# sreeramkannan/Shannon

Hardware: AMD Instinct MI355X
Metric: reads/sec k-mer->graph->path-decompose, 2x100bp k=25 (higher is better)
Workload: dtype u64

## Files before the change

### shannon_amd/csrc/common.h

```cpp
#pragma once
#include <hip/hip_runtime.h>
#include <stdint.h>
#include <stdlib.h>
#include <string>
#include <vector>
#include <mutex>
#include "../../include/shannon_hip.h"

hipError_t shn_counted_memcpy(const char* file, int line, void* dst, const void* src, size_t n, hipMemcpyKind kind, hipStream_t s);
hipError_t shn_counted_memset(const char* file, int line, void* dst, int value, size_t n, hipStream_t s);
#define hipMemcpyAsync(...) shn_counted_memcpy(__FILE__, __LINE__, __VA_ARGS__)
#define hipMemsetAsync(...) shn_counted_memset(__FILE__, __LINE__, __VA_ARGS__)

#define SHN_WAVE 64

static inline const char* shn_env_str(const char* name) { return getenv(name); }
static inline bool shn_env_set(const char* name) { return shn_env_str(name) != nullptr; }
static inline bool shn_env_flag(const char* name, bool dflt) {
  const char* v = shn_env_str(name);
  return !v ? dflt : dflt ? v[0] != '0' : v[0] == '1';
}
static inline uint64_t shn_env_u64(const char* name, uint64_t dflt, uint64_t lo = 0, uint64_t hi = ~0ULL) {
  const char* v = shn_env_str(name);
  if (!v) return dflt;
// ... 323 lines not shown
                   int bit_lo, int bit_hi);

int shn_sort_keys(shn_ctx* ctx, uint64_t* keys, uint64_t* keys_tmp, uint64_t n, int bit_lo, int bit_hi, uint64_t** sorted);

static inline uint64_t cdiv(uint64_t a, uint64_t b) { return (a + b - 1) / b; }

struct ShnDevBufs {
  std::vector<void*> p;
  hipStream_t stream;
  explicit ShnDevBufs(hipStream_t s) : stream(s) {}
  template <class T> hipError_t get(T** out, size_t bytes) { hipError_t e = shn_dev_malloc_on((void**)out, bytes, stream); if (e == hipSuccess) p.push_back((void*)*out); return e; }
  ~ShnDevBufs() { for (void* q : p) shn_dev_free_on(q, stream); }
};
void shn_contig_ids(hipStream_t s, const uint64_t* d_off, uint64_t n_contigs, uint32_t* d_cid);
int shn_sorted_windows(shn_ctx* ctx, ShnDevBufs& bufs, const uint8_t* d_bases, const uint64_t* d_off, const uint32_t* d_cid, const int32_t* d_use,
                       uint64_t total, int k, uint64_t** keys, uint32_t** vals, uint64_t* n_out);
```

### shannon_amd/csrc/contig_gpu.hip

```cpp
#include "contig_graph.h"
#include <atomic>
#include <mutex>

namespace {

#define CG_BLK 256

__global__ void cg_cid_kernel(const uint64_t* __restrict__ off, uint64_t n_cand, uint32_t* __restrict__ cid) {
  const uint64_t c = ((uint64_t)blockIdx.x * blockDim.x + threadIdx.x) >> 6;
  if (c >= n_cand) return;
  const uint64_t lo = off[c], hi = off[c + 1];
  for (uint64_t g = lo + (threadIdx.x & 63); g < hi; g += 64) cid[g] = (uint32_t)c;
}

__global__ void cg_flag_kernel(const uint8_t* __restrict__ bases, const uint64_t* __restrict__ off, const uint32_t* __restrict__ cid,
                               const int32_t* __restrict__ use, uint64_t total, int k, uint32_t* __restrict__ flag) {
  for (uint64_t g = (uint64_t)blockIdx.x * blockDim.x + threadIdx.x; g < total; g += (uint64_t)gridDim.x * blockDim.x) {
    const uint32_t c = cid[g];
    flag[g] = (g + (uint64_t)k <= off[c + 1] && (!use || use[c] != 0)) ? 1u : 0u;
  }
}

__device__ __forceinline__ uint32_t cg_code(uint8_t b) { return b == 'A' ? 0u : b == 'C' ? 1u : b == 'G' ? 2u : b == 'T' ? 3u : 4u; }

__global__ void cg_keys_kernel(const uint8_t* __restrict__ bases, const uint32_t* __restrict__ flag, const uint64_t* __restrict__ pos,
                               uint64_t total, int k, uint64_t* __restrict__ keys, uint32_t* __restrict__ vals,
                               unsigned long long* __restrict__ n_bad) {
  for (uint64_t g = (uint64_t)blockIdx.x * blockDim.x + threadIdx.x; g < total; g += (uint64_t)gridDim.x * blockDim.x) {
    if (!flag[g]) continue;
    uint64_t key = 0;
    bool bad = false;
    for (int j = 0; j < k; j++) { const uint32_t c = cg_code(bases[g + j]); bad |= c > 3; key = (key << 2) | (uint64_t)(c & 3); }
// ... 246 lines not shown
    const uint32_t f = (e - i > 1 && cid[(uint32_t)w] != cid[(uint32_t)last]) ? 1u : 0u;
    for (uint64_t j = i; j < e; j++) flag[j] = f;
  }
}
__global__ void cg_compact_packed_kernel(const uint64_t* __restrict__ words, const uint32_t* __restrict__ flag, const uint64_t* __restrict__ pos, uint64_t n,
                                         uint64_t* __restrict__ okeys, uint32_t* __restrict__ ovals) {
  for (uint64_t i = (uint64_t)blockIdx.x * blockDim.x + threadIdx.x; i < n; i += (uint64_t)gridDim.x * blockDim.x)
    if (flag[i]) { const uint64_t w = words[i]; okeys[pos[i]] = w >> 32; ovals[pos[i]] = (uint32_t)w; }
}
__global__ void cg_compact_kernel(const uint64_t* __restrict__ keys, const uint32_t* __restrict__ vals, const uint32_t* __restrict__ flag,
                                  const uint64_t* __restrict__ pos, uint64_t n, uint64_t* __restrict__ okeys, uint32_t* __restrict__ ovals) {
  for (uint64_t i = (uint64_t)blockIdx.x * blockDim.x + threadIdx.x; i < n; i += (uint64_t)gridDim.x * blockDim.x)
    if (flag[i]) { okeys[pos[i]] = keys[i]; ovals[pos[i]] = vals[i]; }
}

static inline uint32_t grid_for(uint64_t n) { return (uint32_t)std::min<uint64_t>(std::max<uint64_t>(cdiv(n, CG_BLK), 1), 1u << 20); }

}

void shn_contig_ids(hipStream_t s, const uint64_t* d_off, uint64_t n_contigs, uint32_t* d_cid) {
  if (n_contigs) hipLaunchKernelGGL(cg_cid_kernel, dim3((uint32_t)cdiv(n_contigs * 64, CG_BLK)), dim3(CG_BLK), 0, s, d_off, n_contigs, d_cid);
}

int shn_sorted_windows(shn_ctx* ctx, ShnDevBufs& bufs, const uint8_t* d_bases, const uint64_t* d_off, const uint32_t* d_cid,
                          const int32_t* d_use, uint64_t total, int k, uint64_t** keys, uint32_t** vals, uint64_t* n_out) {
  hipStream_t s = ctx->stream; shn_use_stream(s);
  uint32_t* d_flag; uint64_t* d_pos; unsigned long long* d_bad;
  HIP_TRY(bufs.get(&d_flag, (total + 1) * 4));
  HIP_TRY(bufs.get(&d_pos, (total + 2) * 8));
  HIP_TRY(bufs.get(&d_bad, 8));
  HIP_TRY(hipMemsetAsync(d_bad, 0, 8, s));
  hipLaunchKernelGGL(cg_flag_kernel, dim3(grid_for(total)), dim3(CG_BLK), 0, s, d_bases, d_off, d_cid, d_use, total, k, d_flag);
  uint64_t nv = 0;
  int rc = shn_device_scan_u32(ctx, d_flag, total, d_pos, &nv);
  if (rc) return rc;
  *n_out = nv;
  *keys = nullptr; *vals = nullptr;
  if (!nv) return SHN_OK;
  uint64_t *k1, *k2; uint32_t *v1, *v2;
  HIP_TRY(bufs.get(&k1, nv * 8)); HIP_TRY(bufs.get(&k2, nv * 8)); HIP_TRY(bufs.get(&v1, nv * 4)); HIP_TRY(bufs.get(&v2, nv * 4));
  hipLaunchKernelGGL(cg_keys_kernel, dim3(grid_for(total)), dim3(CG_BLK), 0, s, d_bases, d_flag, d_pos, total, k, k1, v1, d_bad);
  unsigned long long bad = 0;
  HIP_TRY(hipMemcpyAsync(&bad, d_bad, 8, hipMemcpyDeviceToHost, s));
  HIP_TRY(hipStreamSynchronize(s));
  if (bad) return shn_fail(SHN_ERR_ARG, "shn_contig_stage: contig with a base outside ACGT");
  if ((rc = shn_sort_pairs(ctx, k1, v1, k2, v2, nv, 0, 2 * k))) return rc;
  *keys = k1; *vals = v1;
  return SHN_OK;
}

static int sorted_windows_packed(shn_ctx* ctx, ShnDevBufs& bufs, const uint8_t* d_bases, const uint64_t* d_off, const uint32_t* d_cid, uint64_t total, int k,
                                 uint64_t** words, uint64_t* n_out) {
  hipStream_t s = ctx->stream; shn_use_stream(s);
  uint32_t* d_flag; uint64_t* d_pos; unsigned long long* d_bad;
  HIP_TRY(bufs.get(&d_flag, (total + 1) * 4));
  HIP_TRY(bufs.get(&d_pos, (total + 2) * 8));
  HIP_TRY(bufs.get(&d_bad, 8));
  HIP_TRY(hipMemsetAsync(d_bad, 0, 8, s));
  hipLaunchKernelGGL(cg_flag_kernel, dim3(grid_for(total)), dim3(CG_BLK), 0, s, d_bases, d_off, d_cid, (const int32_t*)nullptr, total, k, d_flag);
  uint64_t nv = 0;
  int rc = shn_device_scan_u32(ctx, d_flag, total, d_pos, &nv);
  if (rc) return rc;
  *n_out = nv;
  *words = nullptr;
  if (!nv) return SHN_OK;
  uint64_t *w1, *w2;
  HIP_TRY(bufs.get(&w1, nv * 8)); HIP_TRY(bufs.get(&w2, nv * 8));
  hipLaunchKernelGGL(cg_keys_packed_kernel, dim3(grid_for(total)), dim3(CG_BLK), 0, s, d_bases, d_flag, d_pos, total, k, w1, d_bad);
  unsigned long long bad = 0;
  HIP_TRY(hipMemcpyAsync(&bad, d_bad, 8, hipMemcpyDeviceToHost, s));
  HIP_TRY(hipStreamSynchronize(s));
  if (bad) return shn_fail(SHN_ERR_ARG, "shn_contig_stage: contig with a base outside ACGT");
  return shn_sort_keys(ctx, w1, w2, nv, 32, 32 + 2 * k, words);
}
// ... 34 lines not shown
  uint32_t max_len = 0;
  for (uint64_t c = 0; c < n_cand; c++) max_len = std::max<uint32_t>(max_len, (uint32_t)(off[c + 1] - off[c]));
  if (n_cand >= (1u << 21) || max_len >= (1u << 21)) {
    std::vector<uint8_t> fetched;
    if (!bases) {
      fetched.resize(total);
      HIP_TRY(hipMemcpyAsync(fetched.data(), d_bases, total, hipMemcpyDeviceToHost, s));
      HIP_TRY(hipStreamSynchronize(s));
      bases = fetched.data();
    }
    G->add(bases, off, n_cand, accepted_out, best_counts_out);
    *out = G; guard.g = nullptr;
    return SHN_OK;
  }
  uint64_t n_rounds = 0, n_blocks = 0, n_list_rounds = 0;
  {
    ShnDevBufs tmp(s);
    uint64_t* keys = nullptr; uint32_t* vals = nullptr; uint64_t* words = nullptr; uint64_t nv = 0;
    int rc;
    const bool shared_only = shn_env_flag("SHN_CONTIG_SHARED", true);
    const bool packed = r <= 16 && shared_only && shn_env_flag("SHN_CONTIG_PACKED", true);
    { TimerRegion ts(ctx, T_CG_SORT);
      rc = packed ? sorted_windows_packed(ctx, tmp, d_bases, d_off, d_cid, total, r, &words, &nv)
                  : shn_sorted_windows(ctx, tmp, d_bases, d_off, d_cid, nullptr, total, r, &keys, &vals, &nv);
      ts.bytes(packed ? nv * (1 + 8 + (uint64_t)((2 * r + 7) / 8) * 16) : nv * (1 + 12 + (uint64_t)((2 * r + 7) / 8) * 24)); }
    if (rc) return rc;
    lap("r-mer sort (GPU)");
    if (nv > 1 && shared_only) {
      uint32_t* d_f0; uint64_t* d_p0; uint64_t ns0 = 0;
      ShnDevBufs scratch(s);
      HIP_TRY(scratch.get(&d_f0, (nv + 1) * 4));
      HIP_TRY(scratch.get(&d_p0, (nv + 2) * 8));
      if (packed) hipLaunchKernelGGL(cg_shared_packed_kernel, dim3(grid_for(nv)), dim3(CG_BLK), 0, s, words, nv, d_cid, d_f0);
      else hipLaunchKernelGGL(cg_shared_kernel, dim3(grid_for(nv)), dim3(CG_BLK), 0, s, keys, vals, nv, d_cid, d_f0);
      if ((rc = shn_device_scan_u32(ctx, d_f0, nv, d_p0, &ns0))) return rc;
      uint64_t* ok = nullptr; uint32_t* ov = nullptr;
      HIP_TRY(tmp.get(&ok, (ns0 + 1) * 8)); HIP_TRY(tmp.get(&ov, (ns0 + 1) * 4));
      if (ns0 && packed) hipLaunchKernelGGL(cg_compact_packed_kernel, dim3(grid_for(nv)), dim3(CG_BLK), 0, s, words, d_f0, d_p0, nv, ok, ov);
      else if (ns0) hipLaunchKernelGGL(cg_compact_kernel, dim3(grid_for(nv)), dim3(CG_BLK), 0, s, keys, vals, d_f0, d_p0, nv, ok, ov);
      if (dbg) fprintf(stderr, "[contig_stage]   %llu of %llu r-mer windows lie in runs that span two candidates\n", (unsigned long long)ns0, (unsigned long long)nv);
      keys = ok; vals = ov; nv = ns0;
      lap("shared r-mer runs (GPU)");
    } else if (packed && nv == 1) {
      nv = 0;
    }
    uint8_t *d_acc, *d_hit; uint32_t *d_scid, *d_flag, *d_acand, *d_cov, *d_ovf; uint64_t *d_apos, *d_akey; int32_t* d_bestc;
    unsigned long long *d_best, *d_chg;
    HIP_TRY(tmp.get(&d_acc, n_cand + 1)); HIP_TRY(tmp.get(&d_hit, total + 64)); HIP_TRY(tmp.get(&d_scid, (nv + 1) * 4));
    HIP_TRY(tmp.get(&d_flag, (nv + 1) * 4)); HIP_TRY(tmp.get(&d_acand, (nv + 1) * 4)); HIP_TRY(tmp.get(&d_cov, (n_cand + 1) * 4));
    HIP_TRY(tmp.get(&d_ovf, 64)); HIP_TRY(tmp.get(&d_apos, (nv + 2) * 8)); HIP_TRY(tmp.get(&d_akey, (nv + 1) * 8));
    HIP_TRY(tmp.get(&d_bestc, (n_cand + 1) * 4)); HIP_TRY(tmp.get(&d_best, (n_cand + 1) * 8)); HIP_TRY(tmp.get(&d_chg, 64));
    uint8_t *d_aff, *d_chgf; uint32_t* d_aval;
    HIP_TRY(tmp.get(&d_aval, (nv + 1) * 4));
    HIP_TRY(tmp.get(&d_aff, n_cand + 1)); HIP_TRY(tmp.get(&d_chgf, n_cand + 1));
    HIP_TRY(hipMemsetAsync(d_chgf, 0, n_cand + 1, s));
    const bool incremental = shn_env_u64("SHN_CONTIG_INCREMENTAL", 1) != 0;
    HIP_TRY(hipMemsetAsync(d_acc, 0, n_cand + 1, s));
    HIP_TRY(hipMemsetAsync(d_bestc, 0, (n_cand + 1) * 4, s));
    if (nv) hipLaunchKernelGGL(cg_scid_kernel, dim3(grid_for(nv)), dim3(CG_BLK), 0, s, vals, d_cid, nv, d_scid);
    const uint64_t list_max = shn_env_u64("SHN_CONTIG_LIST_MAX", 20000);
    uint32_t *d_pos_of = nullptr, *d_clist = nullptr, *d_alist = nullptr, *d_nlist = nullptr;
    if (list_max && nv && nv < 0xFFFFFFF0ULL) {
      HIP_TRY(tmp.get(&d_pos_of, (total + 1) * 4)); HIP_TRY(tmp.get(&d_clist, (n_cand + 1) * 4)); HIP_TRY(tmp.get(&d_alist, (n_cand + 1) * 4)); HIP_TRY(tmp.get(&d_nlist, 64));
      HIP_TRY(hipMemsetAsync(d_pos_of, 0xFF, (total + 1) * 4, s));
      hipLaunchKernelGGL(cg_pos_of_kernel, dim3(grid_for(nv)), dim3(CG_BLK), 0, s, vals, nv, d_pos_of);
    }
    int lg_slots = 22;
    while (lg_slots < 28 && (1ULL << lg_slots) < nv / 4) lg_slots++;
// ... 88 lines not shown
        if (dbg) fprintf(stderr, "[contig_stage]   block [%llu,%llu) round %d: %llu accepted entries, %llu decisions changed\n", (unsigned long long)lo,
                         (unsigned long long)hi, round, (unsigned long long)na, changed);
        if (!changed) break;
        if (round >= max_rounds && hi - lo > 1) {
          HIP_TRY(hipMemsetAsync(d_aff + lo + (hi - lo) / 2, 0, hi - (lo + (hi - lo) / 2), s));
          hi = lo + (hi - lo) / 2;
          HIP_TRY(hipMemsetAsync(d_acc + hi, 0, n_cand - hi, s));
          HIP_TRY(hipMemsetAsync(d_aff + lo, 1, hi - lo, s));
          round = 0;
        }
      }
      n_blocks++;
      lo = hi;
      bsize = std::min<uint64_t>(bsize * 2, std::max<uint64_t>(blk0, n_cand / 4));
    }
    HIP_TRY(hipMemcpyAsync(acc.data(), d_acc, n_cand, hipMemcpyDeviceToHost, s));
    HIP_TRY(hipMemcpyAsync(best_counts_out, d_bestc, n_cand * 4, hipMemcpyDeviceToHost, s));
    HIP_TRY(hipStreamSynchronize(s));
  }
  std::vector<int32_t> use(n_cand);
  int32_t n_acc = 0;
  for (uint64_t c = 0; c < n_cand; c++) { use[c] = acc[c] ? ++n_acc : 0; accepted_out[c] = use[c]; }
  if (dbg) fprintf(stderr, "[contig_stage] %llu candidates (%llu bases): %llu blocks, %llu rounds (%llu of them candidate by candidate), accepted %d\n",
                   (unsigned long long)n_cand, (unsigned long long)total, (unsigned long long)n_blocks, (unsigned long long)n_rounds, (unsigned long long)n_list_rounds, n_acc);
  lap("duplicate_check rounds (GPU)");

  G->idx = n_acc;
  G->conns.assign((size_t)n_acc + 1, Conn());
  G->n_cand_total = n_cand;
  const int C = k1 - 1;
  if (n_acc > 1) {
    int32_t* d_use;
    HIP_TRY(bufs.get(&d_use, n_cand * 4));
    HIP_TRY(hipMemcpyAsync(d_use, use.data(), n_cand * 4, hipMemcpyHostToDevice, s));
    ShnDevBufs tmp(s);
    uint64_t* keys; uint32_t* vals; uint64_t nv = 0;
    int rc = shn_sorted_windows(ctx, tmp, d_bases, d_off, d_cid, d_use, total, C, &keys, &vals, &nv);
    if (rc) return rc;
    uint64_t ns = 0;
    std::vector<uint64_t> hk; std::vector<uint32_t> hg;
    if (nv > 1) {
      uint32_t* d_flag; uint64_t* d_pos;
      HIP_TRY(tmp.get(&d_flag, (nv + 1) * 4));
      HIP_TRY(tmp.get(&d_pos, (nv + 2) * 8));
      hipLaunchKernelGGL(cg_shared_kernel, dim3(grid_for(nv)), dim3(CG_BLK), 0, s, keys, vals, nv, d_cid, d_flag);
      if ((rc = shn_device_scan_u32(ctx, d_flag, nv, d_pos, &ns))) return rc;
      if (ns) {
        uint64_t* ok; uint32_t* ov;
        HIP_TRY(tmp.get(&ok, ns * 8)); HIP_TRY(tmp.get(&ov, ns * 4));
        hipLaunchKernelGGL(cg_compact_kernel, dim3(grid_for(nv)), dim3(CG_BLK), 0, s, keys, vals, d_flag, d_pos, nv, ok, ov);
        hk.resize(ns); hg.resize(ns);
        HIP_TRY(hipMemcpyAsync(hk.data(), ok, ns * 8, hipMemcpyDeviceToHost, s));
        HIP_TRY(hipMemcpyAsync(hg.data(), ov, ns * 4, hipMemcpyDeviceToHost, s));
        HIP_TRY(hipStreamSynchronize(s));
      }
    }
    if (dbg) fprintf(stderr, "[contig_stage]   %llu of %llu K-mer windows of the accepted contigs lie in runs that span two of them\n", (unsigned long long)ns, (unsigned long long)nv);
    lap("K-mer sort + shared runs (GPU)");
    if (ns) {
      std::vector<uint32_t> run(ns), ea(ns), ep(ns), run_start;
      for (uint64_t e = 0; e < ns; e++) {
        if (e == 0 || hk[e] != hk[e - 1]) run_start.push_back((uint32_t)e);
        run[e] = (uint32_t)run_start.size() - 1;
      }
      run_start.push_back((uint32_t)ns);
      std::vector<uint32_t> order(ns), order2(ns);
      {
        for (uint64_t e = 0; e < ns; e++) order[e] = (uint32_t)e;
        std::vector<uint32_t> cnt(2049);
        for (int pass = 0; pass < 3; pass++) {
          const int sh = 11 * pass;
          if (sh && (total >> sh) == 0) break;
// ... 97 lines not shown
```

### shannon_amd/csrc/probe_gpu.hip

```cpp
#include "common.h"
#include "runs.h"
#include <algorithm>
#include <cstring>
#include <map>

#define PG_BLK 256

struct shn_probe {
  shn_table* table = nullptr;
  std::vector<uint32_t> set_off, set_mem;
};

namespace {

__global__ void pg_head_kernel(const uint64_t* __restrict__ keys, const uint32_t* __restrict__ vals, const uint32_t* __restrict__ cid,
                               const uint32_t* __restrict__ part_of, uint64_t n, uint32_t* __restrict__ head, uint32_t* __restrict__ multi) {
  SHN_GRID_FOR(i, n) {
    if (i && keys[i] == keys[i - 1]) { head[i] = 0; multi[i] = 0; continue; }
    head[i] = 1;
    uint64_t e = i + 1;
    while (e < n && keys[e] == keys[i]) e++;
    multi[i] = part_of[cid[vals[i]]] != part_of[cid[vals[e - 1]]] ? 1u : 0u;
  }
}
// ... 38 lines not shown
                                const uint32_t* __restrict__ part_of, const uint32_t* __restrict__ multi, const uint64_t* __restrict__ hpos,
                                uint64_t n, unsigned long long* __restrict__ n_out, uint64_t cap, uint32_t* __restrict__ o_uidx, uint32_t* __restrict__ o_part) {
  SHN_GRID_FOR(i, n) {
    if (!multi[i]) continue;
    uint32_t p1 = 0, p2 = 0;
    if (pg_run_parts(keys, vals, cid, part_of, n, i, p1, p2) < 3) continue;
    for (uint64_t e = i; e < n && keys[e] == keys[i]; e++) {
      const unsigned long long at = atomicAdd(n_out, 1ULL);
      if (at < cap) { o_uidx[at] = (uint32_t)hpos[i]; o_part[at] = part_of[cid[vals[e]]]; }
    }
  }
}
__global__ void pg_patch_kernel(const uint32_t* __restrict__ uidx, const uint32_t* __restrict__ setid, uint64_t n, uint32_t* __restrict__ uvals) {
  SHN_GRID_FOR(i, n) uvals[uidx[i]] = setid[i] + 1;
}
}

extern "C" void shn_probe_destroy(shn_probe* p) { if (p) { shn_table_destroy(p->table); delete p; } }
extern "C" const shn_table* shn_probe_table(const shn_probe* p) { return p ? p->table : nullptr; }
extern "C" uint32_t shn_probe_n_sets(const shn_probe* p) { return p ? (uint32_t)(p->set_off.size() - 1) : 0; }
extern "C" uint64_t shn_probe_n_members(const shn_probe* p) { return p ? p->set_mem.size() : 0; }
extern "C" int shn_probe_sets(const shn_probe* p, uint32_t* set_off, uint32_t* set_mem) {
  if (!p || !set_off || !set_mem) return shn_fail(SHN_ERR_ARG, "shn_probe_sets: NULL argument");
  std::copy(p->set_off.begin(), p->set_off.end(), set_off);
  std::copy(p->set_mem.begin(), p->set_mem.end(), set_mem);
  return SHN_OK;
}

extern "C" int shn_probe_build(shn_ctx* ctx, const uint8_t* bases, const uint64_t* off, uint64_t n_contigs, const uint32_t* part_of, uint32_t n_parts,
                               int k1, shn_probe** out) {
  if (!ctx || !out || (n_contigs && (!bases || !off || !part_of)) || k1 < 2 || k1 > 32) return shn_fail(SHN_ERR_ARG, "shn_probe_build: bad argument");
  *out = nullptr;
  const uint64_t total = n_contigs ? off[n_contigs] : 0;
  if (total >= 0xFFFFFFF0ULL) return shn_fail(SHN_ERR_OVERFLOW, "shn_probe_build: more than 2^32 contig bases");
  for (uint64_t c = 0; c < n_contigs; c++)
    if (part_of[c] >= n_parts || (c && part_of[c] < part_of[c - 1])) return shn_fail(SHN_ERR_ARG, "shn_probe_build: part_of must be ascending and < n_parts");
  SHN_ENTER(ctx);
  shn_stage_begin(ctx);
  hipStream_t s = ctx->stream;
  shn_probe* P = new shn_probe();
  struct Guard { shn_probe* p; ~Guard() { shn_probe_destroy(p); } } guard{P};
  P->set_off.resize(n_parts + 1);
  P->set_mem.resize(n_parts);
  for (uint32_t p = 0; p <= n_parts; p++) P->set_off[p] = p;
  for (uint32_t p = 0; p < n_parts; p++) P->set_mem[p] = p;
  ShnDevBufs B(ctx->stream);
  uint64_t* ukeys = nullptr; uint32_t* uvals = nullptr;
  uint64_t nu = 0;
  if (total) {
    uint8_t* d_bases; uint64_t* d_off; uint32_t *d_cid, *d_part;
    HIP_TRY(B.get(&d_bases, total + 64)); HIP_TRY(B.get(&d_off, (n_contigs + 1) * 8)); HIP_TRY(B.get(&d_cid, (total + 1) * 4)); HIP_TRY(B.get(&d_part, n_contigs * 4));
    HIP_TRY(hipMemcpyAsync(d_bases, bases, total, hipMemcpyHostToDevice, s));
    HIP_TRY(hipMemcpyAsync(d_off, off, (n_contigs + 1) * 8, hipMemcpyHostToDevice, s));
    HIP_TRY(hipMemcpyAsync(d_part, part_of, n_contigs * 4, hipMemcpyHostToDevice, s));
    shn_contig_ids(s, d_off, n_contigs, d_cid);
    uint64_t* keys; uint32_t* vals; uint64_t nv = 0;
    int rc = shn_sorted_windows(ctx, B, d_bases, d_off, d_cid, nullptr, total, k1, &keys, &vals, &nv);
    if (rc) return rc;
    if (nv) {
      uint32_t *d_head, *d_multi; uint64_t *d_hpos;
      HIP_TRY(B.get(&d_head, (nv + 1) * 4)); HIP_TRY(B.get(&d_multi, (nv + 1) * 4)); HIP_TRY(B.get(&d_hpos, (nv + 2) * 8));
      hipLaunchKernelGGL(pg_head_kernel, dim3(shn_grid(nv, PG_BLK)), dim3(PG_BLK), 0, s, keys, vals, d_cid, d_part, nv, d_head, d_multi);
      if ((rc = shn_device_scan_u32(ctx, d_head, nv, d_hpos, &nu))) return rc;
      HIP_TRY(B.get(&ukeys, (nu + 1) * 8)); HIP_TRY(B.get(&uvals, (nu + 1) * 4));
      hipLaunchKernelGGL(pg_unique_kernel, dim3(shn_grid(nv, PG_BLK)), dim3(PG_BLK), 0, s, keys, vals, d_cid, d_part, d_head, d_hpos, nv, ukeys, uvals);
      unsigned long long* d_nm; uint32_t *d_mu = nullptr, *d_mp = nullptr;
      HIP_TRY(B.get(&d_nm, 8));
      {
        uint64_t *d_pair, *d_pair2, *d_dist; uint32_t *d_pu, *d_pu2;
        HIP_TRY(B.get(&d_pair, (nu + 1) * 8)); HIP_TRY(B.get(&d_pair2, (nu + 1) * 8)); HIP_TRY(B.get(&d_pu, (nu + 1) * 4)); HIP_TRY(B.get(&d_pu2, (nu + 1) * 4));
        HIP_TRY(hipMemsetAsync(d_nm, 0, 8, s));
        hipLaunchKernelGGL(pg_pair_kernel, dim3(shn_grid(nv, PG_BLK)), dim3(PG_BLK), 0, s, keys, vals, d_cid, d_part, d_multi, d_hpos, nv, d_nm, d_pair, d_pu);
        unsigned long long n_pair = 0;
        HIP_TRY(hipMemcpyAsync(&n_pair, d_nm, 8, hipMemcpyDeviceToHost, s));
        HIP_TRY(hipStreamSynchronize(s));
        if (n_pair) {
          if ((rc = shn_sort_pairs(ctx, d_pair, d_pu, d_pair2, d_pu2, n_pair, 0, 32 + shn_bits_for(n_parts)))) return rc;
          ShnRuns runs;
          if ((rc = shn_sorted_runs(ctx, B, d_pair, n_pair, 0, 0, &runs))) return rc;
          const uint64_t n_dist = runs.n_runs;
          HIP_TRY(B.get(&d_dist, (n_dist + 1) * 8));
          const uint32_t first_sid = (uint32_t)(P->set_off.size() - 1);
          hipLaunchKernelGGL(pg_pair_patch_kernel, dim3(shn_grid(n_pair, PG_BLK)), dim3(PG_BLK), 0, s, d_pair, d_pu, runs.head, runs.pos, (uint64_t)n_pair, first_sid, uvals, d_dist);
          std::vector<uint64_t> dist(n_dist);
          HIP_TRY(hipMemcpyAsync(dist.data(), d_dist, n_dist * 8, hipMemcpyDeviceToHost, s));
          HIP_TRY(hipStreamSynchronize(s));
          for (uint64_t pr : dist) {
            P->set_mem.push_back((uint32_t)(pr >> 32)); P->set_mem.push_back((uint32_t)pr);
            P->set_off.push_back((uint32_t)P->set_mem.size());
          }
        }
      }
      uint64_t cap = 1 << 16;
      unsigned long long nm = 0;
      while (true) {
        HIP_TRY(B.get(&d_mu, cap * 4)); HIP_TRY(B.get(&d_mp, cap * 4));
        HIP_TRY(hipMemsetAsync(d_nm, 0, 8, s));
        hipLaunchKernelGGL(pg_multi_kernel, dim3(shn_grid(nv, PG_BLK)), dim3(PG_BLK), 0, s, keys, vals, d_cid, d_part, d_multi, d_hpos, nv, d_nm, cap, d_mu, d_mp);
        HIP_TRY(hipMemcpyAsync(&nm, d_nm, 8, hipMemcpyDeviceToHost, s));
        HIP_TRY(hipStreamSynchronize(s));
        if (nm <= cap) break;
        cap = nm;
      }
      if (nm) {
        std::vector<uint32_t> mu(nm), mp(nm);
        HIP_TRY(hipMemcpy(mu.data(), d_mu, nm * 4, hipMemcpyDeviceToHost));
        HIP_TRY(hipMemcpy(mp.data(), d_mp, nm * 4, hipMemcpyDeviceToHost));
        std::vector<uint32_t> order(nm);
        for (uint64_t i = 0; i < nm; i++) order[i] = (uint32_t)i;
        std::sort(order.begin(), order.end(), [&](uint32_t a, uint32_t b) { return mu[a] != mu[b] ? mu[a] < mu[b] : mp[a] < mp[b]; });
        std::map<std::vector<uint32_t>, uint32_t> ids;
        std::vector<uint32_t> pu, ps, cur;
        for (uint64_t i = 0; i < nm;) {
          const uint32_t u = mu[order[i]];
          cur.clear();
          for (; i < nm && mu[order[i]] == u; i++) if (cur.empty() || cur.back() != mp[order[i]]) cur.push_back(mp[order[i]]);
          auto it = ids.find(cur);
          uint32_t sid;
          if (it != ids.end()) sid = it->second;
          else {
            sid = (uint32_t)(P->set_off.size() - 1);
            ids[cur] = sid;
            P->set_mem.insert(P->set_mem.end(), cur.begin(), cur.end());
            P->set_off.push_back((uint32_t)P->set_mem.size());
          }
          pu.push_back(u); ps.push_back(sid);
        }
        uint32_t *d_pu, *d_ps;
        HIP_TRY(B.get(&d_pu, pu.size() * 4)); HIP_TRY(B.get(&d_ps, ps.size() * 4));
        HIP_TRY(hipMemcpyAsync(d_pu, pu.data(), pu.size() * 4, hipMemcpyHostToDevice, s));
        HIP_TRY(hipMemcpyAsync(d_ps, ps.data(), ps.size() * 4, hipMemcpyHostToDevice, s));
        hipLaunchKernelGGL(pg_patch_kernel, dim3(shn_grid(pu.size(), PG_BLK)), dim3(PG_BLK), 0, s, d_pu, d_ps, (uint64_t)pu.size(), uvals);
        HIP_TRY(hipStreamSynchronize(s));
      }
    }
  }
  if (!ukeys) { HIP_TRY(B.get(&ukeys, 8)); HIP_TRY(B.get(&uvals, 4)); }
  int rc = shn_table_from_pairs(ctx, ukeys, uvals, nu, k1, 0, &P->table);
  if (rc) return rc;
  HIP_TRY(hipStreamSynchronize(s));
  HIP_TRY(hipGetLastError());
  *out = P;
  guard.p = nullptr;
  return SHN_OK;
}
```

Before: 67.86 million.

## Restrict K-mer join to shared-run windows and skip probe sort when k-mers are distinct

The contig stage keeps the shared r-mer runs of accepted candidates and uses them to select only the windows that can share a K-mer across contigs before the full K-mer sort. This avoids sorting every window of every accepted contig. The probe build first hashes contig ends on the host to detect repeated contigs. If none are found, it builds the lookup table directly from unsorted window pairs and falls back to the sorted path only if some k1-mer repeats. Both changes add extra passes, a host-side hash check and longer buffer lifetimes, and the window selection rests on the assumption that any shared K-mer implies a shared r-mer run.

After: 62.82 million. -7.4%, worse.

```diff
diff --git a/shannon_amd/csrc/common.h b/shannon_amd/csrc/common.h
--- a/shannon_amd/csrc/common.h
+++ b/shannon_amd/csrc/common.h
@@ -361,4 +361,4 @@
 };
 void shn_contig_ids(hipStream_t s, const uint64_t* d_off, uint64_t n_contigs, uint32_t* d_cid);
 int shn_sorted_windows(shn_ctx* ctx, ShnDevBufs& bufs, const uint8_t* d_bases, const uint64_t* d_off, const uint32_t* d_cid, const int32_t* d_use,
-                       uint64_t total, int k, uint64_t** keys, uint32_t** vals, uint64_t* n_out);
+                       const uint8_t* d_sel, uint64_t total, int k, uint64_t** keys, uint32_t** vals, uint64_t* n_out);
diff --git a/shannon_amd/csrc/contig_gpu.hip b/shannon_amd/csrc/contig_gpu.hip
--- a/shannon_amd/csrc/contig_gpu.hip
+++ b/shannon_amd/csrc/contig_gpu.hip
@@ -1,5 +1,6 @@
 #include "contig_graph.h"
 #include <atomic>
+#include <memory>
 #include <mutex>
 
 namespace {
@@ -14,8 +15,9 @@
 }
 
 __global__ void cg_flag_kernel(const uint8_t* __restrict__ bases, const uint64_t* __restrict__ off, const uint32_t* __restrict__ cid,
-                               const int32_t* __restrict__ use, uint64_t total, int k, uint32_t* __restrict__ flag) {
+                               const int32_t* __restrict__ use, const uint8_t* __restrict__ sel, uint64_t total, int k, uint32_t* __restrict__ flag) {
   for (uint64_t g = (uint64_t)blockIdx.x * blockDim.x + threadIdx.x; g < total; g += (uint64_t)gridDim.x * blockDim.x) {
+    if (sel && sel[g] == 0) { flag[g] = 0; continue; }
     const uint32_t c = cid[g];
     flag[g] = (g + (uint64_t)k <= off[c + 1] && (!use || use[c] != 0)) ? 1u : 0u;
   }
@@ -292,6 +294,24 @@
     if (flag[i]) { okeys[pos[i]] = keys[i]; ovals[pos[i]] = vals[i]; }
 }
 
+__global__ void cg_join_select_kernel(const uint64_t* __restrict__ akey, const uint32_t* __restrict__ acand, const uint32_t* __restrict__ aval, uint64_t na,
+                                      const uint64_t* __restrict__ off, int C, uint8_t* __restrict__ sel) {
+  for (uint64_t i = (uint64_t)blockIdx.x * blockDim.x + threadIdx.x; i < na; i += (uint64_t)gridDim.x * blockDim.x) {
+    const uint32_t c = acand[i], g = aval[i];
+    if ((uint64_t)g + (uint64_t)C > off[c + 1]) continue;
+    const uint64_t key = akey[i];
+    uint64_t j = i;
+    while (j > 0 && akey[j - 1] == key && acand[j - 1] == c) j--;
+    bool other = j > 0 && akey[j - 1] == key;
+    if (!other) {
+      j = i + 1;
+      while (j < na && akey[j] == key && acand[j] == c) j++;
+      other = j < na && akey[j] == key;
+    }
+    if (other) sel[g] = 1;
+  }
+}
+
 static inline uint32_t grid_for(uint64_t n) { return (uint32_t)std::min<uint64_t>(std::max<uint64_t>(cdiv(n, CG_BLK), 1), 1u << 20); }
 
 }
@@ -301,14 +321,14 @@
 }
 
 int shn_sorted_windows(shn_ctx* ctx, ShnDevBufs& bufs, const uint8_t* d_bases, const uint64_t* d_off, const uint32_t* d_cid,
-                          const int32_t* d_use, uint64_t total, int k, uint64_t** keys, uint32_t** vals, uint64_t* n_out) {
+                          const int32_t* d_use, const uint8_t* d_sel, uint64_t total, int k, uint64_t** keys, uint32_t** vals, uint64_t* n_out) {
   hipStream_t s = ctx->stream; shn_use_stream(s);
   uint32_t* d_flag; uint64_t* d_pos; unsigned long long* d_bad;
   HIP_TRY(bufs.get(&d_flag, (total + 1) * 4));
   HIP_TRY(bufs.get(&d_pos, (total + 2) * 8));
   HIP_TRY(bufs.get(&d_bad, 8));
   HIP_TRY(hipMemsetAsync(d_bad, 0, 8, s));
-  hipLaunchKernelGGL(cg_flag_kernel, dim3(grid_for(total)), dim3(CG_BLK), 0, s, d_bases, d_off, d_cid, d_use, total, k, d_flag);
+  hipLaunchKernelGGL(cg_flag_kernel, dim3(grid_for(total)), dim3(CG_BLK), 0, s, d_bases, d_off, d_cid, d_use, d_sel, total, k, d_flag);
   uint64_t nv = 0;
   int rc = shn_device_scan_u32(ctx, d_flag, total, d_pos, &nv);
   if (rc) return rc;
@@ -335,7 +355,7 @@
   HIP_TRY(bufs.get(&d_pos, (total + 2) * 8));
   HIP_TRY(bufs.get(&d_bad, 8));
   HIP_TRY(hipMemsetAsync(d_bad, 0, 8, s));
-  hipLaunchKernelGGL(cg_flag_kernel, dim3(grid_for(total)), dim3(CG_BLK), 0, s, d_bases, d_off, d_cid, (const int32_t*)nullptr, total, k, d_flag);
+  hipLaunchKernelGGL(cg_flag_kernel, dim3(grid_for(total)), dim3(CG_BLK), 0, s, d_bases, d_off, d_cid, (const int32_t*)nullptr, (const uint8_t*)nullptr, total, k, d_flag);
   uint64_t nv = 0;
   int rc = shn_device_scan_u32(ctx, d_flag, total, d_pos, &nv);
   if (rc) return rc;
@@ -400,15 +420,19 @@
     return SHN_OK;
   }
   uint64_t n_rounds = 0, n_blocks = 0, n_list_rounds = 0;
+  const bool join_list = r <= k1 - 1 && !shn_env_flag("SHN_CONTIG_JOIN_ALL", false);
+  std::unique_ptr<ShnDevBufs> keep(new ShnDevBufs(s));
+  uint64_t* sh_keys = nullptr; uint32_t *sh_cand = nullptr, *sh_vals = nullptr; uint64_t sh_n = 0;
   {
     ShnDevBufs tmp(s);
     uint64_t* keys = nullptr; uint32_t* vals = nullptr; uint64_t* words = nullptr; uint64_t nv = 0;
+    bool have_list = false;
     int rc;
     const bool shared_only = shn_env_flag("SHN_CONTIG_SHARED", true);
     const bool packed = r <= 16 && shared_only && shn_env_flag("SHN_CONTIG_PACKED", true);
     { TimerRegion ts(ctx, T_CG_SORT);
       rc = packed ? sorted_windows_packed(ctx, tmp, d_bases, d_off, d_cid, total, r, &words, &nv)
-                  : shn_sorted_windows(ctx, tmp, d_bases, d_off, d_cid, nullptr, total, r, &keys, &vals, &nv);
+                  : shn_sorted_windows(ctx, tmp, d_bases, d_off, d_cid, nullptr, nullptr, total, r, &keys, &vals, &nv);
       ts.bytes(packed ? nv * (1 + 8 + (uint64_t)((2 * r + 7) / 8) * 16) : nv * (1 + 12 + (uint64_t)((2 * r + 7) / 8) * 24)); }
     if (rc) return rc;
     lap("r-mer sort (GPU)");
@@ -426,6 +450,7 @@
       else if (ns0) hipLaunchKernelGGL(cg_compact_kernel, dim3(grid_for(nv)), dim3(CG_BLK), 0, s, keys, vals, d_f0, d_p0, nv, ok, ov);
       if (dbg) fprintf(stderr, "[contig_stage]   %llu of %llu r-mer windows lie in runs that span two candidates\n", (unsigned long long)ns0, (unsigned long long)nv);
       keys = ok; vals = ov; nv = ns0;
+      have_list = true;
       lap("shared r-mer runs (GPU)");
     } else if (packed && nv == 1) {
       nv = 0;
@@ -433,11 +458,12 @@
     uint8_t *d_acc, *d_hit; uint32_t *d_scid, *d_flag, *d_acand, *d_cov, *d_ovf; uint64_t *d_apos, *d_akey; int32_t* d_bestc;
     unsigned long long *d_best, *d_chg;
     HIP_TRY(tmp.get(&d_acc, n_cand + 1)); HIP_TRY(tmp.get(&d_hit, total + 64)); HIP_TRY(tmp.get(&d_scid, (nv + 1) * 4));
-    HIP_TRY(tmp.get(&d_flag, (nv + 1) * 4)); HIP_TRY(tmp.get(&d_acand, (nv + 1) * 4)); HIP_TRY(tmp.get(&d_cov, (n_cand + 1) * 4));
-    HIP_TRY(tmp.get(&d_ovf, 64)); HIP_TRY(tmp.get(&d_apos, (nv + 2) * 8)); HIP_TRY(tmp.get(&d_akey, (nv + 1) * 8));
+    ShnDevBufs& ib = join_list && have_list ? *keep : tmp;
+    HIP_TRY(tmp.get(&d_flag, (nv + 1) * 4)); HIP_TRY(ib.get(&d_acand, (nv + 1) * 4)); HIP_TRY(tmp.get(&d_cov, (n_cand + 1) * 4));
+    HIP_TRY(tmp.get(&d_ovf, 64)); HIP_TRY(tmp.get(&d_apos, (nv + 2) * 8)); HIP_TRY(ib.get(&d_akey, (nv + 1) * 8));
     HIP_TRY(tmp.get(&d_bestc, (n_cand + 1) * 4)); HIP_TRY(tmp.get(&d_best, (n_cand + 1) * 8)); HIP_TRY(tmp.get(&d_chg, 64));
     uint8_t *d_aff, *d_chgf; uint32_t* d_aval;
-    HIP_TRY(tmp.get(&d_aval, (nv + 1) * 4));
+    HIP_TRY(ib.get(&d_aval, (nv + 1) * 4));
     HIP_TRY(tmp.get(&d_aff, n_cand + 1)); HIP_TRY(tmp.get(&d_chgf, n_cand + 1));
     HIP_TRY(hipMemsetAsync(d_chgf, 0, n_cand + 1, s));
     const bool incremental = shn_env_u64("SHN_CONTIG_INCREMENTAL", 1) != 0;
@@ -556,6 +582,15 @@
       lo = hi;
       bsize = std::min<uint64_t>(bsize * 2, std::max<uint64_t>(blk0, n_cand / 4));
     }
+    if (dbg) HIP_TRY(hipStreamSynchronize(s));
+    lap("duplicate_check rounds (GPU)");
+    if (join_list && have_list && nv) {
+      hipLaunchKernelGGL(cg_accflag_kernel, dim3(grid_for(nv)), dim3(CG_BLK), 0, s, d_scid, d_acc, nv, (uint32_t)n_cand, (uint32_t)n_cand, d_flag);
+      if ((rc = shn_device_scan_u32(ctx, d_flag, nv, d_apos, &sh_n))) return rc;
+      if (sh_n) hipLaunchKernelGGL(cg_acc_compact_kernel, dim3(grid_for(nv)), dim3(CG_BLK), 0, s, keys, d_scid, d_flag, vals, d_apos, nv, d_akey, d_acand, d_aval);
+      sh_keys = d_akey; sh_cand = d_acand; sh_vals = d_aval;
+      if (dbg) fprintf(stderr, "[contig_stage]   %llu of the %llu shared r-mer entries belong to accepted candidates\n", (unsigned long long)sh_n, (unsigned long long)nv);
+    }
     HIP_TRY(hipMemcpyAsync(acc.data(), d_acc, n_cand, hipMemcpyDeviceToHost, s));
     HIP_TRY(hipMemcpyAsync(best_counts_out, d_bestc, n_cand * 4, hipMemcpyDeviceToHost, s));
     HIP_TRY(hipStreamSynchronize(s));
@@ -565,7 +600,7 @@
   for (uint64_t c = 0; c < n_cand; c++) { use[c] = acc[c] ? ++n_acc : 0; accepted_out[c] = use[c]; }
   if (dbg) fprintf(stderr, "[contig_stage] %llu candidates (%llu bases): %llu blocks, %llu rounds (%llu of them candidate by candidate), accepted %d\n",
                    (unsigned long long)n_cand, (unsigned long long)total, (unsigned long long)n_blocks, (unsigned long long)n_rounds, (unsigned long long)n_list_rounds, n_acc);
-  lap("duplicate_check rounds (GPU)");
+  lap("accepted shared entries, decisions");
 
   G->idx = n_acc;
   G->conns.assign((size_t)n_acc + 1, Conn());
@@ -576,8 +611,17 @@
     HIP_TRY(bufs.get(&d_use, n_cand * 4));
     HIP_TRY(hipMemcpyAsync(d_use, use.data(), n_cand * 4, hipMemcpyHostToDevice, s));
     ShnDevBufs tmp(s);
+    uint8_t* d_sel = nullptr;
+    if (join_list && sh_n) {
+      HIP_TRY(tmp.get(&d_sel, total + 1));
+      HIP_TRY(hipMemsetAsync(d_sel, 0, total + 1, s));
+      hipLaunchKernelGGL(cg_join_select_kernel, dim3(grid_for(sh_n)), dim3(CG_BLK), 0, s, sh_keys, sh_cand, sh_vals, sh_n, d_off, C, d_sel);
+      if (dbg) { HIP_TRY(hipStreamSynchronize(s)); fprintf(stderr, "[contig_stage]   K-mer join: windows selected from %llu accepted entries of the shared r-mer runs\n", (unsigned long long)sh_n); }
+      lap("join windows from shared runs (GPU)");
+    }
+    keep.reset();
     uint64_t* keys; uint32_t* vals; uint64_t nv = 0;
-    int rc = shn_sorted_windows(ctx, tmp, d_bases, d_off, d_cid, d_use, total, C, &keys, &vals, &nv);
+    int rc = shn_sorted_windows(ctx, tmp, d_bases, d_off, d_cid, d_use, d_sel, total, C, &keys, &vals, &nv);
     if (rc) return rc;
     uint64_t ns = 0;
     std::vector<uint64_t> hk; std::vector<uint32_t> hg;
@@ -597,7 +641,7 @@
         HIP_TRY(hipStreamSynchronize(s));
       }
     }
-    if (dbg) fprintf(stderr, "[contig_stage]   %llu of %llu K-mer windows of the accepted contigs lie in runs that span two of them\n", (unsigned long long)ns, (unsigned long long)nv);
+    if (dbg) fprintf(stderr, "[contig_stage]   %llu of %llu sorted K-mer windows of the accepted contigs lie in runs that span two of them\n", (unsigned long long)ns, (unsigned long long)nv);
     lap("K-mer sort + shared runs (GPU)");
     if (ns) {
       std::vector<uint32_t> run(ns), ea(ns), ep(ns), run_start;
diff --git a/shannon_amd/csrc/probe_gpu.hip b/shannon_amd/csrc/probe_gpu.hip
--- a/shannon_amd/csrc/probe_gpu.hip
+++ b/shannon_amd/csrc/probe_gpu.hip
@@ -1,6 +1,8 @@
 #include "common.h"
 #include "runs.h"
 #include <algorithm>
+#include <chrono>
+#include <cstdio>
 #include <cstring>
 #include <map>
 
@@ -76,6 +78,53 @@
 __global__ void pg_patch_kernel(const uint32_t* __restrict__ uidx, const uint32_t* __restrict__ setid, uint64_t n, uint32_t* __restrict__ uvals) {
   SHN_GRID_FOR(i, n) uvals[uidx[i]] = setid[i] + 1;
 }
+
+__device__ __forceinline__ uint32_t pg_code(uint8_t b) { return b == 'A' ? 0u : b == 'C' ? 1u : b == 'G' ? 2u : b == 'T' ? 3u : 4u; }
+__global__ void pg_direct_kernel(const uint8_t* __restrict__ bases, const uint64_t* __restrict__ off, const uint64_t* __restrict__ woff,
+                                 const uint32_t* __restrict__ cid, const uint32_t* __restrict__ part_of, uint64_t total, int k,
+                                 uint64_t* __restrict__ keys, uint32_t* __restrict__ vals, unsigned long long* __restrict__ n_bad) {
+  SHN_GRID_FOR(g, total) {
+    const uint32_t c = cid[g];
+    if (g + (uint64_t)k > off[c + 1]) continue;
+    uint64_t key = 0;
+    bool bad = false;
+    for (int j = 0; j < k; j++) { const uint32_t b = pg_code(bases[g + j]); bad |= b > 3; key = (key << 2) | (uint64_t)(b & 3); }
+    if (bad) atomicAdd(n_bad, 1ULL);
+    const uint64_t at = woff[c] + (g - off[c]);
+    keys[at] = key;
+    vals[at] = part_of[c] + 1;
+  }
+}
+
+static bool pg_contigs_repeat(const uint8_t* bases, const uint64_t* off, uint64_t n_contigs, int k) {
+  std::vector<uint64_t> h;
+  h.reserve(n_contigs);
+  for (uint64_t c = 0; c < n_contigs; c++) {
+    if (c + 17 <= n_contigs && off[c + 17] - off[c + 16] >= 32) {
+      const uint8_t *a = bases + off[c + 16], *z = bases + off[c + 17];
+      __builtin_prefetch(a); __builtin_prefetch(a + 31); __builtin_prefetch(z - 32); __builtin_prefetch(z - 1);
+    }
+    const uint64_t len = off[c + 1] - off[c];
+    if (len < (uint64_t)k) continue;
+    const uint64_t m = std::min<uint64_t>(len, 32);
+    uint64_t w[8] = {0, 0, 0, 0, 0, 0, 0, 0};
+    memcpy(w, bases + off[c], m);
+    memcpy(w + 4, bases + off[c + 1] - m, m);
+    uint64_t x = shn_mix64(len);
+    for (int j = 0; j < 8; j++) x = shn_mix64(x ^ w[j]);
+    h.push_back(x ? x : 1);
+  }
+  uint64_t slots = 16;
+  while (slots < 2 * h.size()) slots <<= 1;
+  std::vector<uint64_t> tab(slots, 0);
+  for (uint64_t x : h) {
+    uint64_t s = x & (slots - 1);
+    while (tab[s] && tab[s] != x) s = (s + 1) & (slots - 1);
+    if (tab[s]) return true;
+    tab[s] = x;
+  }
+  return false;
+}
 }
 
 extern "C" void shn_probe_destroy(shn_probe* p) { if (p) { shn_table_destroy(p->table); delete p; } }
@@ -86,6 +135,94 @@
   if (!p || !set_off || !set_mem) return shn_fail(SHN_ERR_ARG, "shn_probe_sets: NULL argument");
   std::copy(p->set_off.begin(), p->set_off.end(), set_off);
   std::copy(p->set_mem.begin(), p->set_mem.end(), set_mem);
+  return SHN_OK;
+}
+
+static int probe_sorted_pairs(shn_ctx* ctx, shn_probe* P, ShnDevBufs& B, const uint8_t* d_bases, const uint64_t* d_off, const uint32_t* d_cid,
+                              const uint32_t* d_part, uint64_t total, uint32_t n_parts, int k1, uint64_t** ukeys_out, uint32_t** uvals_out, uint64_t* nu_out) {
+  hipStream_t s = ctx->stream;
+  uint64_t* ukeys = nullptr; uint32_t* uvals = nullptr; uint64_t nu = 0;
+  uint64_t* keys; uint32_t* vals; uint64_t nv = 0;
+  int rc = shn_sorted_windows(ctx, B, d_bases, d_off, d_cid, nullptr, nullptr, total, k1, &keys, &vals, &nv);
+  if (rc) return rc;
+  if (nv) {
+    uint32_t *d_head, *d_multi; uint64_t *d_hpos;
+    HIP_TRY(B.get(&d_head, (nv + 1) * 4)); HIP_TRY(B.get(&d_multi, (nv + 1) * 4)); HIP_TRY(B.get(&d_hpos, (nv + 2) * 8));
+    hipLaunchKernelGGL(pg_head_kernel, dim3(shn_grid(nv, PG_BLK)), dim3(PG_BLK), 0, s, keys, vals, d_cid, d_part, nv, d_head, d_multi);
+    if ((rc = shn_device_scan_u32(ctx, d_head, nv, d_hpos, &nu))) return rc;
+    HIP_TRY(B.get(&ukeys, (nu + 1) * 8)); HIP_TRY(B.get(&uvals, (nu + 1) * 4));
+    hipLaunchKernelGGL(pg_unique_kernel, dim3(shn_grid(nv, PG_BLK)), dim3(PG_BLK), 0, s, keys, vals, d_cid, d_part, d_head, d_hpos, nv, ukeys, uvals);
+    unsigned long long* d_nm; uint32_t *d_mu = nullptr, *d_mp = nullptr;
+    HIP_TRY(B.get(&d_nm, 8));
+    {
+      uint64_t *d_pair, *d_pair2, *d_dist; uint32_t *d_pu, *d_pu2;
+      HIP_TRY(B.get(&d_pair, (nu + 1) * 8)); HIP_TRY(B.get(&d_pair2, (nu + 1) * 8)); HIP_TRY(B.get(&d_pu, (nu + 1) * 4)); HIP_TRY(B.get(&d_pu2, (nu + 1) * 4));
+      HIP_TRY(hipMemsetAsync(d_nm, 0, 8, s));
+      hipLaunchKernelGGL(pg_pair_kernel, dim3(shn_grid(nv, PG_BLK)), dim3(PG_BLK), 0, s, keys, vals, d_cid, d_part, d_multi, d_hpos, nv, d_nm, d_pair, d_pu);
+      unsigned long long n_pair = 0;
+      HIP_TRY(hipMemcpyAsync(&n_pair, d_nm, 8, hipMemcpyDeviceToHost, s));
+      HIP_TRY(hipStreamSynchronize(s));
+      if (n_pair) {
+        if ((rc = shn_sort_pairs(ctx, d_pair, d_pu, d_pair2, d_pu2, n_pair, 0, 32 + shn_bits_for(n_parts)))) return rc;
+        ShnRuns runs;
+        if ((rc = shn_sorted_runs(ctx, B, d_pair, n_pair, 0, 0, &runs))) return rc;
+        const uint64_t n_dist = runs.n_runs;
+        HIP_TRY(B.get(&d_dist, (n_dist + 1) * 8));
+        const uint32_t first_sid = (uint32_t)(P->set_off.size() - 1);
+        hipLaunchKernelGGL(pg_pair_patch_kernel, dim3(shn_grid(n_pair, PG_BLK)), dim3(PG_BLK), 0, s, d_pair, d_pu, runs.head, runs.pos, (uint64_t)n_pair, first_sid, uvals, d_dist);
+        std::vector<uint64_t> dist(n_dist);
+        HIP_TRY(hipMemcpyAsync(dist.data(), d_dist, n_dist * 8, hipMemcpyDeviceToHost, s));
+        HIP_TRY(hipStreamSynchronize(s));
+        for (uint64_t pr : dist) {
+          P->set_mem.push_back((uint32_t)(pr >> 32)); P->set_mem.push_back((uint32_t)pr);
+          P->set_off.push_back((uint32_t)P->set_mem.size());
+        }
+      }
+    }
+    uint64_t cap = 1 << 16;
+    unsigned long long nm = 0;
+    while (true) {
+      HIP_TRY(B.get(&d_mu, cap * 4)); HIP_TRY(B.get(&d_mp, cap * 4));
+      HIP_TRY(hipMemsetAsync(d_nm, 0, 8, s));
+      hipLaunchKernelGGL(pg_multi_kernel, dim3(shn_grid(nv, PG_BLK)), dim3(PG_BLK), 0, s, keys, vals, d_cid, d_part, d_multi, d_hpos, nv, d_nm, cap, d_mu, d_mp);
+      HIP_TRY(hipMemcpyAsync(&nm, d_nm, 8, hipMemcpyDeviceToHost, s));
+      HIP_TRY(hipStreamSynchronize(s));
+      if (nm <= cap) break;
+      cap = nm;
+    }
+    if (nm) {
+      std::vector<uint32_t> mu(nm), mp(nm);
+      HIP_TRY(hipMemcpy(mu.data(), d_mu, nm * 4, hipMemcpyDeviceToHost));
+      HIP_TRY(hipMemcpy(mp.data(), d_mp, nm * 4, hipMemcpyDeviceToHost));
+      std::vector<uint32_t> order(nm);
+      for (uint64_t i = 0; i < nm; i++) order[i] = (uint32_t)i;
+      std::sort(order.begin(), order.end(), [&](uint32_t a, uint32_t b) { return mu[a] != mu[b] ? mu[a] < mu[b] : mp[a] < mp[b]; });
+      std::map<std::vector<uint32_t>, uint32_t> ids;
+      std::vector<uint32_t> pu, ps, cur;
+      for (uint64_t i = 0; i < nm;) {
+        const uint32_t u = mu[order[i]];
+        cur.clear();
+        for (; i < nm && mu[order[i]] == u; i++) if (cur.empty() || cur.back() != mp[order[i]]) cur.push_back(mp[order[i]]);
+        auto it = ids.find(cur);
+        uint32_t sid;
+        if (it != ids.end()) sid = it->second;
+        else {
+          sid = (uint32_t)(P->set_off.size() - 1);
+          ids[cur] = sid;
+          P->set_mem.insert(P->set_mem.end(), cur.begin(), cur.end());
+          P->set_off.push_back((uint32_t)P->set_mem.size());
+        }
+        pu.push_back(u); ps.push_back(sid);
+      }
+      uint32_t *d_pu, *d_ps;
+      HIP_TRY(B.get(&d_pu, pu.size() * 4)); HIP_TRY(B.get(&d_ps, ps.size() * 4));
+      HIP_TRY(hipMemcpyAsync(d_pu, pu.data(), pu.size() * 4, hipMemcpyHostToDevice, s));
+      HIP_TRY(hipMemcpyAsync(d_ps, ps.data(), ps.size() * 4, hipMemcpyHostToDevice, s));
+      hipLaunchKernelGGL(pg_patch_kernel, dim3(shn_grid(pu.size(), PG_BLK)), dim3(PG_BLK), 0, s, d_pu, d_ps, (uint64_t)pu.size(), uvals);
+      HIP_TRY(hipStreamSynchronize(s));
+    }
+  }
+  *ukeys_out = ukeys; *uvals_out = uvals; *nu_out = nu;
   return SHN_OK;
 }
 
@@ -116,86 +253,52 @@
     HIP_TRY(hipMemcpyAsync(d_off, off, (n_contigs + 1) * 8, hipMemcpyHostToDevice, s));
     HIP_TRY(hipMemcpyAsync(d_part, part_of, n_contigs * 4, hipMemcpyHostToDevice, s));
     shn_contig_ids(s, d_off, n_contigs, d_cid);
-    uint64_t* keys; uint32_t* vals; uint64_t nv = 0;
-    int rc = shn_sorted_windows(ctx, B, d_bases, d_off, d_cid, nullptr, total, k1, &keys, &vals, &nv);
-    if (rc) return rc;
-    if (nv) {
-      uint32_t *d_head, *d_multi; uint64_t *d_hpos;
-      HIP_TRY(B.get(&d_head, (nv + 1) * 4)); HIP_TRY(B.get(&d_multi, (nv + 1) * 4)); HIP_TRY(B.get(&d_hpos, (nv + 2) * 8));
-      hipLaunchKernelGGL(pg_head_kernel, dim3(shn_grid(nv, PG_BLK)), dim3(PG_BLK), 0, s, keys, vals, d_cid, d_part, nv, d_head, d_multi);
-      if ((rc = shn_device_scan_u32(ctx, d_head, nv, d_hpos, &nu))) return rc;
-      HIP_TRY(B.get(&ukeys, (nu + 1) * 8)); HIP_TRY(B.get(&uvals, (nu + 1) * 4));
-      hipLaunchKernelGGL(pg_unique_kernel, dim3(shn_grid(nv, PG_BLK)), dim3(PG_BLK), 0, s, keys, vals, d_cid, d_part, d_head, d_hpos, nv, ukeys, uvals);
-      unsigned long long* d_nm; uint32_t *d_mu = nullptr, *d_mp = nullptr;
-      HIP_TRY(B.get(&d_nm, 8));
-      {
-        uint64_t *d_pair, *d_pair2, *d_dist; uint32_t *d_pu, *d_pu2;
-        HIP_TRY(B.get(&d_pair, (nu + 1) * 8)); HIP_TRY(B.get(&d_pair2, (nu + 1) * 8)); HIP_TRY(B.get(&d_pu, (nu + 1) * 4)); HIP_TRY(B.get(&d_pu2, (nu + 1) * 4));
-        HIP_TRY(hipMemsetAsync(d_nm, 0, 8, s));
-        hipLaunchKernelGGL(pg_pair_kernel, dim3(shn_grid(nv, PG_BLK)), dim3(PG_BLK), 0, s, keys, vals, d_cid, d_part, d_multi, d_hpos, nv, d_nm, d_pair, d_pu);
-        unsigned long long n_pair = 0;
-        HIP_TRY(hipMemcpyAsync(&n_pair, d_nm, 8, hipMemcpyDeviceToHost, s));
+    const bool dbg = shn_env_set("SHN_DEBUG");
+    auto now = []() { return std::chrono::duration<double>(std::chrono::steady_clock::now().time_since_epoch()).count(); };
+    double t0 = now();
+    auto lap = [&](const char* what) { if (dbg) { HIP_TRY(hipStreamSynchronize(s)); double t = now(); fprintf(stderr, "[probe_build] %-34s %8.3f s\n", what, t - t0); t0 = t; } return (int)SHN_OK; };
+    lap("upload + contig ids");
+    const bool repeat = shn_env_flag("SHN_PROBE_SORTED", false) || pg_contigs_repeat(bases, off, n_contigs, k1);
+    lap("repeated contigs? (host)");
+    if (!repeat) {
+      std::vector<uint64_t> woff(n_contigs + 1);
+      uint64_t nw = 0;
+      for (uint64_t c = 0; c < n_contigs; c++) { woff[c] = nw; const uint64_t len = off[c + 1] - off[c]; if (len >= (uint64_t)k1) nw += len - (uint64_t)k1 + 1; }
+      woff[n_contigs] = nw;
+      if (nw) {
+        ShnDevBufs D(s);
+        uint64_t *d_woff, *dk; uint32_t* dv; unsigned long long* d_bad;
+        HIP_TRY(D.get(&d_woff, (n_contigs + 1) * 8)); HIP_TRY(D.get(&dk, (nw + 1) * 8)); HIP_TRY(D.get(&dv, (nw + 1) * 4)); HIP_TRY(D.get(&d_bad, 8));
+        HIP_TRY(hipMemcpyAsync(d_woff, woff.data(), (n_contigs + 1) * 8, hipMemcpyHostToDevice, s));
+        HIP_TRY(hipMemsetAsync(d_bad, 0, 8, s));
+        hipLaunchKernelGGL(pg_direct_kernel, dim3(shn_grid(total, PG_BLK)), dim3(PG_BLK), 0, s, d_bases, d_off, d_woff, d_cid, d_part, total, k1, dk, dv, d_bad);
+        unsigned long long bad = 0;
+        HIP_TRY(hipMemcpyAsync(&bad, d_bad, 8, hipMemcpyDeviceToHost, s));
         HIP_TRY(hipStreamSynchronize(s));
-        if (n_pair) {
-          if ((rc = shn_sort_pairs(ctx, d_pair, d_pu, d_pair2, d_pu2, n_pair, 0, 32 + shn_bits_for(n_parts)))) return rc;
-          ShnRuns runs;
-          if ((rc = shn_sorted_runs(ctx, B, d_pair, n_pair, 0, 0, &runs))) return rc;
-          const uint64_t n_dist = runs.n_runs;
-          HIP_TRY(B.get(&d_dist, (n_dist + 1) * 8));
-          const uint32_t first_sid = (uint32_t)(P->set_off.size() - 1);
-          hipLaunchKernelGGL(pg_pair_patch_kernel, dim3(shn_grid(n_pair, PG_BLK)), dim3(PG_BLK), 0, s, d_pair, d_pu, runs.head, runs.pos, (uint64_t)n_pair, first_sid, uvals, d_dist);
-          std::vector<uint64_t> dist(n_dist);
-          HIP_TRY(hipMemcpyAsync(dist.data(), d_dist, n_dist * 8, hipMemcpyDeviceToHost, s));
-          HIP_TRY(hipStreamSynchronize(s));
-          for (uint64_t pr : dist) {
-            P->set_mem.push_back((uint32_t)(pr >> 32)); P->set_mem.push_back((uint32_t)pr);
-            P->set_off.push_back((uint32_t)P->set_mem.size());
-          }
-        }
+        if (bad) return shn_fail(SHN_ERR_ARG, "shn_contig_stage: contig with a base outside ACGT");
+        lap("unsorted pairs (GPU)");
+        int rc = shn_table_from_pairs(ctx, dk, dv, nw, k1, 0, &P->table);
+        if (rc) return rc;
+        lap("table of the unsorted pairs");
+        const bool distinct = shn_table_size(P->table) == nw;
+        if (dbg) fprintf(stderr, "[probe_build] unsorted pairs: %llu windows, %llu distinct k1-mers: %s\n", (unsigned long long)nw,
+                         (unsigned long long)shn_table_size(P->table), distinct ? "kept" : "a k1-mer repeats, sorted path");
+        if (!distinct) { shn_table_destroy(P->table); P->table = nullptr; }
       }
-      uint64_t cap = 1 << 16;
-      unsigned long long nm = 0;
-      while (true) {
-        HIP_TRY(B.get(&d_mu, cap * 4)); HIP_TRY(B.get(&d_mp, cap * 4));
-        HIP_TRY(hipMemsetAsync(d_nm, 0, 8, s));
-        hipLaunchKernelGGL(pg_multi_kernel, dim3(shn_grid(nv, PG_BLK)), dim3(PG_BLK), 0, s, keys, vals, d_cid, d_part, d_multi, d_hpos, nv, d_nm, cap, d_mu, d_mp);
-        HIP_TRY(hipMemcpyAsync(&nm, d_nm, 8, hipMemcpyDeviceToHost, s));
-        HIP_TRY(hipStreamSynchronize(s));
-        if (nm <= cap) break;
-        cap = nm;
-      }
-      if (nm) {
-        std::vector<uint32_t> mu(nm), mp(nm);
-        HIP_TRY(hipMemcpy(mu.data(), d_mu, nm * 4, hipMemcpyDeviceToHost));
-        HIP_TRY(hipMemcpy(mp.data(), d_mp, nm * 4, hipMemcpyDeviceToHost));
-        std::vector<uint32_t> order(nm);
-        for (uint64_t i = 0; i < nm; i++) order[i] = (uint32_t)i;
-        std::sort(order.begin(), order.end(), [&](uint32_t a, uint32_t b) { return mu[a] != mu[b] ? mu[a] < mu[b] : mp[a] < mp[b]; });
-        std::map<std::vector<uint32_t>, uint32_t> ids;
-        std::vector<uint32_t> pu, ps, cur;
-        for (uint64_t i = 0; i < nm;) {
-          const uint32_t u = mu[order[i]];
-          cur.clear();
-          for (; i < nm && mu[order[i]] == u; i++) if (cur.empty() || cur.back() != mp[order[i]]) cur.push_back(mp[order[i]]);
-          auto it = ids.find(cur);
-          uint32_t sid;
-          if (it != ids.end()) sid = it->second;
-          else {
-            sid = (uint32_t)(P->set_off.size() - 1);
-            ids[cur] = sid;
-            P->set_mem.insert(P->set_mem.end(), cur.begin(), cur.end());
-            P->set_off.push_back((uint32_t)P->set_mem.size());
-          }
-          pu.push_back(u); ps.push_back(sid);
-        }
-        uint32_t *d_pu, *d_ps;
-        HIP_TRY(B.get(&d_pu, pu.size() * 4)); HIP_TRY(B.get(&d_ps, ps.size() * 4));
-        HIP_TRY(hipMemcpyAsync(d_pu, pu.data(), pu.size() * 4, hipMemcpyHostToDevice, s));
-        HIP_TRY(hipMemcpyAsync(d_ps, ps.data(), ps.size() * 4, hipMemcpyHostToDevice, s));
-        hipLaunchKernelGGL(pg_patch_kernel, dim3(shn_grid(pu.size(), PG_BLK)), dim3(PG_BLK), 0, s, d_pu, d_ps, (uint64_t)pu.size(), uvals);
-        HIP_TRY(hipStreamSynchronize(s));
-      }
-    }
+    }
+    if (!P->table) {
+      if (dbg) fprintf(stderr, "[probe_build] sorted path\n");
+      int rc = probe_sorted_pairs(ctx, P, B, d_bases, d_off, d_cid, d_part, total, n_parts, k1, &ukeys, &uvals, &nu);
+      if (rc) return rc;
+      lap("sorted windows, run heads, sets");
+    }
+  }
+  if (P->table) {
+    HIP_TRY(hipStreamSynchronize(s));
+    HIP_TRY(hipGetLastError());
+    *out = P;
+    guard.p = nullptr;
+    return SHN_OK;
   }
   if (!ukeys) { HIP_TRY(B.get(&ukeys, 8)); HIP_TRY(B.get(&uvals, 4)); }
   int rc = shn_table_from_pairs(ctx, ukeys, uvals, nu, k1, 0, &P->table);
```
